# TalShor/SciLMM

Measured on AMD Instinct MI355X. Metric: REML factorize+solve nnz(L)/s (simulated pedigree, fp64), higher is better.
Workload: dtype f64

## Files before the change

scilmm_amd/_lib.py:

```python
import ctypes as C
import os

import numpy as np

_HERE = os.path.dirname(os.path.abspath(__file__))
LIB_PATH = os.environ.get("SCILMM_HIP_LIB", os.path.join(_HERE, "csrc", "libscilmm_hip.so"))

OK, ERR_ARG, ERR_NOT_PD, ERR_DEVICE, ERR_STATE = 0, -1, -2, -3, -4
DOSAGE_U16, DOSAGE_F32 = 0, 1


class ScilmmError(RuntimeError):
    pass


class NotPositiveDefiniteError(ScilmmError):

    def __init__(self, column):
        super().__init__("matrix is not positive definite (failing permuted column %d)" % column)
        self.column = column


class Options(C.Structure):
    _fields_ = [("ordering", C.c_int32), ("relax_small", C.c_int32), ("relax_w1", C.c_int32),
# ... 192 lines not shown

def check(status, sym=None, bad_col=None):
    if status == OK:
        return
    if status == ERR_NOT_PD:
        raise NotPositiveDefiniteError(-1 if bad_col is None else int(bad_col))
    msg = {ERR_ARG: "invalid argument", ERR_DEVICE: "HIP device error", ERR_STATE: "invalid call order"}.get(
        status, "error %d" % status)
    if sym:
        detail = lib().scilmm_symbolic_error(sym)
        if detail:
            msg += ": " + detail.decode()
    raise ScilmmError(msg)


def ptr(a):
    return a.ctypes.data_as(C.c_void_p)


_GET_DTYPES = {"sn_rowptr": np.int64, "sn_loff": np.int64, "asm_dst": np.int64, "diag_dst": np.int64,
               "upd_ptr": np.int64, "tile_base": np.int64, "combo_ptr": np.int64, "level_tile_ptr": np.int64,
               "level_pair_ptr": np.int64, "child_ptr": np.int64, "tail_blk_ptr": np.int64, "pat_colptr": np.int64, "inv_off": np.int64,
               "pat_rowptr": np.int64, "pat_rowslot": np.int64, "pull_seg_ptr": np.int64, "pull_level_ptr": np.int64,
               "pull_fold_ptr": np.int64}


def symbolic_get(sym, name):
    n = C.c_int64(0)
    check(lib().scilmm_symbolic_get(sym, name.encode(), None, C.byref(n)), sym)
    out = np.empty(n.value, dtype=np.int64 if name.startswith("val_") else _GET_DTYPES.get(name, np.int32))
    check(lib().scilmm_symbolic_get(sym, name.encode(), ptr(out), C.byref(n)), sym)
    return out


COMM_FN = C.CFUNCTYPE(C.c_int, C.c_void_p, C.c_int32, C.c_int32, C.c_int64, C.c_int64, C.c_int32)

ORDER_METHODS = {"amd": 0, "nesdis": 1, "nesdis_always": 2}


def order(A, method="amd"):
    indptr = np.ascontiguousarray(A.indptr, dtype=np.int64)
    indices = np.ascontiguousarray(A.indices, dtype=np.int32)
    perm = np.empty(A.shape[0], dtype=np.int32)
    check(lib().scilmm_order(A.shape[0], ptr(indptr), ptr(indices), ORDER_METHODS[method], ptr(perm)))
    return perm


# ... 69 lines not shown
```

scilmm_amd/csrc/capi_symbolic.cpp:

```cpp
#include <cstdlib>
#include <cstring>
#include <exception>
#include <memory>
#include <string>
#include <vector>

#include "../../include/scilmm_hip.h"
#include "handles.h"
#include "host_threads.h"

using scilmm::Symbolic;

static bool env_deterministic() {
  const char* e = getenv("SCILMM_DETERMINISTIC");
  return e && e[0] == '1';
}

extern "C" {

int scilmm_symbolic_create(int32_t n, int32_t K, const int64_t* const* indptr, const int32_t* const* indices,
                           const int32_t* perm_in, const scilmm_options* opts, int32_t ngpus, scilmm_symbolic** out) {
  scilmm::use_host_threads();
  if (!out || n < 0 || K <= 0 || !indptr || !indices || ngpus < 1) return SCILMM_ERR_ARG;
  scilmm::SymbolicOptions o;
  if (opts) {
    o.ordering = opts->ordering;
    if (opts->relax_small >= 0) o.relax_small = opts->relax_small;
    if (opts->relax_w1 >= 0) o.relax_w1 = opts->relax_w1;
    if (opts->relax_w2 >= 0) o.relax_w2 = opts->relax_w2;
    if (opts->relax_z1 >= 0) o.relax_z1 = opts->relax_z1;
    if (opts->relax_z2 >= 0) o.relax_z2 = opts->relax_z2;
    if (opts->relax_z3 >= 0) o.relax_z3 = opts->relax_z3;
// ... 110 lines not shown
  try {
    if (!h->S->combos_built && !std::strncmp(what, "combo_", 6)) scilmm::build_tile_combos(h->S, nullptr);
    if (!std::strncmp(what, "pull_", 5)) scilmm::build_pull_schedule(h->S);
    if (!std::strcmp(what, "pat_rowptr") || !std::strcmp(what, "pat_rowslot") || !std::strcmp(what, "pat_rowcol"))
      if (!scilmm::build_row_index(h->S)) return SCILMM_ERR_STATE;
  } catch (const std::exception& e) {
    const_cast<scilmm_symbolic*>(h)->err = e.what();
    return SCILMM_ERR_STATE;
  }
  const Symbolic& S = *h->S;
  if (!std::strcmp(what, "dense_first")) {
    if (out) *(int32_t*)out = S.dense_first;
    *count = 1;
    return SCILMM_OK;
  }
  if (!std::strncmp(what, "val_slot:", 9) || !std::strncmp(what, "val_src:", 8)) {
    const bool slot = what[4] == 's' && what[5] == 'l';
    const int k = std::atoi(what + (slot ? 9 : 8));
    if (k < 0 || k >= S.K) return SCILMM_ERR_ARG;
    const std::vector<int64_t>& v = slot ? S.val_slot[k] : S.val_src[k];
    if (out) std::memcpy(out, v.data(), v.size() * sizeof(int64_t));
    *count = (int64_t)v.size();
    return SCILMM_OK;
  }
  GET("perm", perm)
  GET("iperm", iperm)
  GET("parent", parent)
  GET("colcount", colcount)
  GET("sn_start", sn_start)
  GET("sn_parent", sn_parent)
  GET("sn_rowptr", sn_rowptr)
  GET("sn_rows", sn_rows)
  GET("sn_loff", sn_loff)
  GET("sn_level", sn_level)
  GET("level_ptr", level_ptr)
  GET("level_fronts", level_fronts)
  GET("asm_dst", asm_dst)
  GET("diag_dst", diag_dst)
  GET("upd_ptr", upd_ptr)
  GET("upd_src", upd_src)
  GET("upd_p0", upd_p0)
  GET("upd_p1", upd_p1)
  GET("tile_base", tile_base)
  GET("tile_front", tile_front)
  GET("combo_ptr", combo_ptr)
  GET("combo_pair", combo_pair)
// ... 85 lines not shown
```

scilmm_amd/csrc/dev.h:

```cpp
#pragma once
#include <hip/hip_runtime.h>

#include <algorithm>
#include <cstdlib>
#include <optional>
#include <string>
#include <type_traits>
#include <vector>

#include "../../include/scilmm_hip.h"
#include "plan_types.h"
#include "handles.h"

namespace scilmm {

struct Tuning {
  int reserve_cus = 0;
  int side_streams = 2;
  bool no_mfma = false;
  bool trsm_lite = true;
  std::optional<bool> dense;
  std::optional<bool> outside;
  bool outside_merge = true;
  std::optional<int> outside_chunks;
  bool outside_prio = false;
  std::optional<double> cell_limit;
  bool no_lookahead = false;
  int look_depth = 2;
  bool host_cells = false;
  bool no_splitk = false;
  int64_t target_items = 1024;
  int64_t min_item = 24;
  int64_t max_item = 96;
  std::optional<int64_t> dense_items;
  int64_t dense_fill = 256;
  std::optional<bool> dense_taper;
  std::optional<int> dist_group;
  bool dist_nosplit = false;
  int chain_cap = 2048;
  int chain_wide = 12;
  bool no_chain = false;
  int64_t push_slice = 512;
  bool shadow = true;
  bool dense_feed = true;
  int chain_wide_t = 160;
  int chain_full_t = 768;
  bool chain_pipe = true;
  int chain_stagger = 0;
// ... 6 lines not shown
  const char* gate = getenv("SCILMM_TUNING");
  const char* e = getenv("SCILMM_DENSE_FEED");
  return !(gate && gate[0] == '1' && e && e[0] == '0');
}

inline Tuning read_tuning() {
  Tuning t;
  t.dense_feed = read_dense_feed();
  const char* gate = getenv("SCILMM_TUNING");
  if (!(gate && gate[0] == '1')) return t;
  auto env = [](const char* name) { return getenv(name); };
  auto is1 = [&](const char* name) { const char* e = env(name); return e && e[0] == '1'; };
  auto not0 = [&](const char* name) { const char* e = env(name); return !(e && e[0] == '0'); };
  const char* e;
  if ((e = env("SCILMM_RESERVE_CUS"))) t.reserve_cus = atoi(e);
  if ((e = env("SCILMM_SIDE_STREAMS"))) t.side_streams = atoi(e);
  t.no_mfma = is1("SCILMM_NO_MFMA");
  t.trsm_lite = not0("SCILMM_TRSM_LITE");
  if ((e = env("SCILMM_DENSE"))) t.dense = e[0] != '0';
  if ((e = env("SCILMM_OUTSIDE"))) t.outside = e[0] != '0';
  t.outside_merge = not0("SCILMM_OUTSIDE_MERGE");
  if ((e = env("SCILMM_OUTSIDE_CHUNKS"))) t.outside_chunks = atoi(e);
  t.outside_prio = is1("SCILMM_OUTSIDE_PRIO");
  if ((e = env("SCILMM_CELL_LIMIT"))) t.cell_limit = atof(e);
  t.no_lookahead = is1("SCILMM_NO_LOOKAHEAD");
  if ((e = env("SCILMM_LOOK_DEPTH"))) t.look_depth = std::max(1, atoi(e));
  t.host_cells = is1("SCILMM_HOST_CELLS");
  t.no_splitk = is1("SCILMM_NO_SPLITK");
  if ((e = env("SCILMM_TARGET_ITEMS"))) t.target_items = atoll(e);
  if ((e = env("SCILMM_MIN_ITEM"))) t.min_item = atoll(e);
  if ((e = env("SCILMM_MAX_ITEM"))) t.max_item = atoll(e);
  if ((e = env("SCILMM_DENSE_ITEMS"))) t.dense_items = atoll(e);
  if ((e = env("SCILMM_DENSE_FILL"))) t.dense_fill = atoll(e);
  if ((e = env("SCILMM_DENSE_TAPER"))) t.dense_taper = e[0] == '1';
  if ((e = env("SCILMM_DIST_GROUP"))) t.dist_group = atoi(e);
  t.dist_nosplit = is1("SCILMM_DIST_NOSPLIT");
  if ((e = env("SCILMM_CHAIN_CAP"))) t.chain_cap = atoi(e);
  if ((e = env("SCILMM_CHAIN_WIDE"))) t.chain_wide = atoi(e);
  t.no_chain = is1("SCILMM_NO_CHAIN");
  if ((e = env("SCILMM_PUSH_SLICE"))) t.push_slice = atoll(e);
  t.shadow = not0("SCILMM_SHADOW");
  if ((e = env("SCILMM_CHAIN_WIDE_T"))) t.chain_wide_t = atoi(e);
  if ((e = env("SCILMM_CHAIN_FULL_T"))) t.chain_full_t = atoi(e);
  t.chain_pipe = not0("SCILMM_CHAIN_PIPE");
  if ((e = env("SCILMM_CHAIN_STAGGER"))) t.chain_stagger = std::max(0, atoi(e));
  t.sinv_generic = is1("SCILMM_SINV_GENERIC");
// ... 128 lines not shown
  int32_t* d_col_front = nullptr;
  int64_t* d_yoff = nullptr;
  double* d_ybuf = nullptr;
  int32_t* d_sinv_pre_tiles = nullptr;
  std::vector<int64_t> sinv_pre_ptr;
  std::vector<int32_t> sinv_tail_front;
  int32_t* d_sinv_tail_fronts = nullptr;
  SinvWork* d_sinv_work = nullptr;
  std::vector<int64_t> sinv_work_ptr;
  std::vector<int32_t> sinv_tail_nseg;
  double* d_sinv_tail_partial = nullptr;
  SinvSeg* d_sinv_cc_segs = nullptr;
  std::vector<int64_t> sinv_cc_seg_ptr;
  SinvFold* d_sinv_cc_folds = nullptr;
  std::vector<int64_t> sinv_cc_fold_ptr;
  double* d_sinv_cc_partial = nullptr;
  bool work_external = false;
  bool outside_on = false;
  int32_t tail_level = 0;
  std::vector<uint8_t> outside_desc;
  OutsideWork* d_owork = nullptr;
  int32_t* d_grp_next = nullptr;
  int32_t* d_grp_t0 = nullptr;
  int64_t n_owork = 0;
  int32_t* d_tail_front = nullptr;
  uint8_t* d_keep_front = nullptr;
  hipStream_t outside_st = nullptr;
  std::vector<int64_t> ochunk_ptr;
  std::vector<hipEvent_t> out_evs;
  std::vector<int32_t> out_wait_chunk;
  bool dense_on = false;
  int front_bits = 64;
  double* d_zeros = nullptr;
  DenseWork* d_dwork_e = nullptr;
  DenseWork* d_dwork_l = nullptr;
  std::vector<int64_t> dwork_e_ptr, dwork_l_ptr;
  std::vector<int64_t> dwork_l_mid;
  int64_t n_late_split = 0;
  int look_depth = 2;
  int rhs_pending = -1;
  int32_t chain_T = 0, chain_l0 = 0;
  int32_t* d_chain = nullptr;
  int32_t* d_colmap = nullptr;
  int32_t* d_cf_ptr = nullptr;
  ChainPair* d_cf = nullptr;
  int32_t* d_cb_ptr = nullptr;
// ... 178 lines not shown
```

scilmm_amd/csrc/kernels.hip.h:

```cpp
#pragma once
#include <hip/hip_runtime.h>
#ifndef SCILMM_UPD_WAVES
#define SCILMM_UPD_WAVES 2
#endif
#include <stdint.h>
#include <type_traits>

#include "plan_types.h"

namespace scilmm {

typedef double d4 __attribute__((ext_vector_type(4)));

constexpr int NJB = NB / 16;
constexpr int KCS = 16;
constexpr int LDA = TM + 16;
constexpr int LDB = NB + 16;
constexpr int LDP = 34;

__device__ __forceinline__ d4 mfma_f64(double a, double b, d4 c) {
  return __builtin_amdgcn_mfma_f64_16x16x4f64(a, b, c, 0, 0, 0);
}

__global__ void k_assemble(int64_t nnz, const int64_t* __restrict__ dst, ValPtrs vp, double* __restrict__ L) {
// ... 842 lines not shown
#endif
  double* P = L + S.sn_loff[j];
#pragma unroll
  for (int jb = 0; jb < NJH; ++jb)
#pragma unroll
    for (int ib = 0; ib < 2; ++ib)
#pragma unroll
      for (int r = 0; r < 4; ++r) {
        const int i = ia + ib, jc = 64 * ch + 16 * jb + 4 * lk + r;
#ifdef SCILMM_DENSE_H_NOFOLD
        const double v = (double)c32[jb][ib][r];
#else
        const double v = acc[jb][ib][r];
#endif
        if (slot < 0) {
          if (i < nrow && jc < wj) P[(int64_t)jc * mj + R0 + i] -= v;
        } else {
          scratch[(int64_t)slot * (TM * NB) + jc * TM + i] = v;
        }
      }
}

template <bool MFMA, int SCATTER = 0>
__global__ __launch_bounds__(256) void k_outside(DevSym S, int32_t dense_first, const OutsideWork* __restrict__ work,
                                                 const int32_t* __restrict__ tail_front,
                                                 const uint8_t* __restrict__ keep_front,
                                                 const int32_t* __restrict__ grp_next,
                                                 const int32_t* __restrict__ grp_t0,
                                                 double* __restrict__ L) {
  __shared__ __attribute__((aligned(16))) double As[KCS * LDA];
  __shared__ __attribute__((aligned(16))) double Bs[KCS * LDB];
  __shared__ int32_t lab_i[TM], lab_j[NB];
  const int tid = threadIdx.x, lane = tid & 63, wv = tid >> 6;
  const OutsideWork wk = work[blockIdx.x];
  int32_t ni, nj;
  {
    const int32_t d = wk.d;
    const int32_t md = (int32_t)(S.sn_rowptr[d + 1] - S.sn_rowptr[d]);
    const int32_t* rd = S.sn_rows + S.sn_rowptr[d];
    const int32_t ri0 = wk.t0 + TM * wk.bi, rj0 = wk.t0 + NB * wk.bj;
    ni = min(TM, md - ri0);
    nj = min(NB, md - rj0);
    if (tid < TM) lab_i[tid] = tid < ni ? rd[ri0 + tid] : -1;
    else if (tid < TM + NB) lab_j[tid - TM] = (tid - TM) < nj ? rd[rj0 + tid - TM] : -1;
  }
  d4 acc[NJB][2];
#pragma unroll
  for (int a = 0; a < NJB; ++a) { acc[a][0] = (d4){0.0, 0.0, 0.0, 0.0}; acc[a][1] = (d4){0.0, 0.0, 0.0, 0.0}; }
  const int x = tid & 127, kk = tid >> 7;
  bool first_chunk = true;
  for (int32_t d = wk.d, t0 = wk.t0; d >= 0;) {
    const int32_t wd = S.sn_start[d + 1] - S.sn_start[d];
    const int32_t md = (int32_t)(S.sn_rowptr[d + 1] - S.sn_rowptr[d]);
    const double* Pd = L + S.sn_loff[d];
    const int32_t ri0 = t0 + TM * wk.bi, rj0 = t0 + NB * wk.bj;
    const double* pa = Pd + ri0 + min(x, ni - 1);
    const double* pb = Pd + rj0 + min(x, nj - 1);
    for (int32_t k0 = 0; k0 < wd; k0 += KCS) {
      const int kc = min(KCS, wd - k0);
      const int kc4 = (kc + 3) & ~3;
      double va[KCS / 2], vb[KCS / 2];
#pragma unroll
      for (int i = 0; i < KCS / 2; ++i) {
        const int64_t kq = k0 + min(kk + 2 * i, kc - 1);
        va[i] = pa[kq * md];
        vb[i] = pb[kq * md];
      }
      if (!first_chunk) __syncthreads();
      first_chunk = false;
#pragma unroll
      for (int i = 0; i < KCS / 2; ++i) {
        const int k = kk + 2 * i;
        if (k < kc4) {
          As[k * LDA + x] = (x < ni && k < kc) ? va[i] : 0.0;
          Bs[k * LDB + x] = (x < nj && k < kc) ? vb[i] : 0.0;
        }
      }
      __syncthreads();
      if (32 * wv < ni) tile_mma<MFMA>(As, Bs, kc4, NJB, lane, wv, acc);
    }
    d = grp_next[d];
    if (d >= 0) t0 = grp_t0[d];
  }
  const int li = lane & 15, lr = lane >> 4;
  const int32_t c0_tail = S.sn_start[dense_first];
#pragma unroll
  for (int jb = 0; jb < NJB; ++jb)
#pragma unroll
    for (int r = 0; r < 4; ++r) {
      const int jloc = 16 * jb + lr + 4 * r;
      const int32_t cj = lab_j[jloc];
      if (cj < 0) continue;
      const int32_t f = tail_front[cj - c0_tail];
      if (!keep_front[f]) continue;
      const int32_t c0f = S.sn_start[f];
      double* col = L + S.sn_loff[f] + (int64_t)(cj - c0f) * (S.n - c0f) - c0f;
#pragma unroll
      for (int ib = 0; ib < 2; ++ib) {
        const int iloc = 32 * wv + 16 * ib + li;
        const int32_t ci = lab_i[iloc];
        if (SCATTER == 0) {
          if (ci >= cj) unsafeAtomicAdd(col + ci, -acc[jb][ib][r]);
        } else if (SCATTER == 1) {
          if (ci >= cj && acc[jb][ib][r] == 123.456) col[ci] = 0.0;
        } else {
          if (ci >= cj) col[ci] = -acc[jb][ib][r];
        }
      }
    }
}


__device__ __forceinline__ double cell_dot(const double* __restrict__ L, int64_t st, int64_t sq, int64_t md, int wd) {
  const double* pt = L + st;
  const double* pq = L + sq;
  double acc = 0.0;
  int k = 0;
  for (; k + 8 <= wd; k += 8) {
    double a[8], b[8];
#pragma unroll
    for (int u = 0; u < 8; ++u) {
      a[u] = pt[(int64_t)(k + u) * md];
      b[u] = pq[(int64_t)(k + u) * md];
    }
    double s0 = 0.0, s1 = 0.0;
#pragma unroll
    for (int u = 0; u < 8; u += 2) {
      s0 += a[u] * b[u];
      s1 += a[u + 1] * b[u + 1];
    }
    acc += s0 + s1;
  }
// ... 2356 lines not shown
```

scilmm_amd/csrc/launch.hip.h:

```cpp
#pragma once

namespace {

int set_attrs(scilmm_symbolic* sym, Dev* D) {
  if (D->attrs_set) return SCILMM_OK;
  const int big = 150 * 1024;
  HIPCHK(hipFuncSetAttribute((const void*)k_potrf, hipFuncAttributeMaxDynamicSharedMemorySize, big));
  HIPCHK(hipFuncSetAttribute((const void*)k_fwd<true, 0, true>, hipFuncAttributeMaxDynamicSharedMemorySize, big));
  HIPCHK(hipFuncSetAttribute((const void*)k_fwd<true, 0, false>, hipFuncAttributeMaxDynamicSharedMemorySize, big));
  HIPCHK(hipFuncSetAttribute((const void*)k_fwd<true, 1, true>, hipFuncAttributeMaxDynamicSharedMemorySize, big));
  HIPCHK(hipFuncSetAttribute((const void*)k_fwd<false, 0, true>, hipFuncAttributeMaxDynamicSharedMemorySize, big));
  HIPCHK(hipFuncSetAttribute((const void*)k_fwd<false, 0, false>, hipFuncAttributeMaxDynamicSharedMemorySize, big));
  HIPCHK(hipFuncSetAttribute((const void*)k_fwd<false, 1, true>, hipFuncAttributeMaxDynamicSharedMemorySize, big));
  HIPCHK(hipFuncSetAttribute((const void*)k_dense32, hipFuncAttributeMaxDynamicSharedMemorySize, big));
  HIPCHK(hipFuncSetAttribute((const void*)k_dense_h, hipFuncAttributeMaxDynamicSharedMemorySize, big));
  HIPCHK(hipFuncSetAttribute((const void*)k_dense_b<2>, hipFuncAttributeMaxDynamicSharedMemorySize, big));
  HIPCHK(hipFuncSetAttribute((const void*)k_dense_b<0>, hipFuncAttributeMaxDynamicSharedMemorySize, big));
  HIPCHK(hipFuncSetAttribute((const void*)k_update2<true>, hipFuncAttributeMaxDynamicSharedMemorySize, big));
  HIPCHK(hipFuncSetAttribute((const void*)k_update2<false>, hipFuncAttributeMaxDynamicSharedMemorySize, big));
  D->attrs_set = true;
  return SCILMM_OK;
}

inline int64_t max_groups(unsigned threads) { return (int64_t)(((uint64_t)1 << 32) / threads) - 1; }
// ... 62 lines not shown
                       (const int32_t*)CS.wd, fac->L);
    launches++;
    return SCILMM_OK;
  }

  void trsm(hipStream_t stream, const int32_t* tiles, int64_t cnt, const double* slabs) {
    const bool lite = D->use_mfma && D->trsm_lite;
    const auto k = lite ? k_trsm_lite : D->use_mfma ? k_trsm<true> : k_trsm<false>;
    const int64_t per = lite ? max_groups(256) / 4 : max_groups(256);
    for (int64_t o = 0; o < cnt; o += per) {
      const int64_t c = std::min(cnt - o, per);
      hipLaunchKernelGGL(k, dim3((unsigned)(lite ? 4 * c : c)), dim3(256), 0, stream, D->v, tiles + o, fac->L, fac->invD, D->d_tile_pslot,
                         D->d_tile_pnseg, slabs);
      launches++;
    }
  }

  void outside(hipStream_t stream, const OutsideWork* work, int64_t cnt) {
    auto k = D->use_mfma ? k_outside<true> : k_outside<false>;
#ifdef SCILMM_DIAG
    if (D->ablate == 6) k = k_outside<true, 1>;
    if (D->ablate == 7) k = k_outside<true, 2>;
#endif
    for (int64_t o = 0; o < cnt; o += max_groups(256)) {
      const unsigned c = (unsigned)std::min<int64_t>(max_groups(256), cnt - o);
      hipLaunchKernelGGL(k, dim3(c), dim3(256), 0, stream, D->v, fac->sym->S->dense_first, work + o, D->d_tail_front, D->d_keep_front,
                         D->d_grp_next, D->d_grp_t0, fac->L);
      launches++;
      D->n_float_atomic++;
    }
  }
};

struct SweepLaunch {
  Dev* const D;
  const scilmm_factor* const fac;
  const hipStream_t st;
  int rp = 0;
  unsigned gy = 1;

  void diag_solve(bool trans, const int32_t* fronts, int64_t cnt, const double* in, double* out) const {
    if (cnt <= 0) return;
    const auto k = D->use_mfma ? (trans ? k_diag_solve<true, true> : k_diag_solve<true, false>)
                               : (trans ? k_diag_solve<false, true> : k_diag_solve<false, false>);
    hipLaunchKernelGGL(k, dim3((unsigned)cnt, gy), dim3(256), 0, st, D->v, fronts, fac->invD, in, out, rp);
  }

  void fwd(int mode, bool atomic, const int32_t* tiles, int64_t cnt, const double* in, double* out) const {
    if (cnt <= 0) return;
    const size_t sm_fwd = sizeof(double) * (size_t)(NB * LDW + KCS * LDA);
// ... 87 lines not shown
```

scilmm_amd/csrc/plan.hip:

```cpp
#include <hip/hip_runtime.h>

#include <algorithm>
#include <atomic>
#include <chrono>
#include <functional>
#include <thread>
#include <cmath>
#include <cstdio>
#include <cstdlib>
#include <cstring>
#include <string>
#include <vector>

#include "dev.h"
#include "cellplan.hip.h"
#include "host_threads.h"

namespace scilmm {

void dev_free(void* p) {
  Dev* D = (Dev*)p;
  if (!D) return;
  for (void* a : D->allocs) (void)hipFree(a);
  for (double* v : D->vals)
// ... 390 lines not shown
  const Symbolic& S = *sym->S;
  const int32_t tail_w = tail_width(S);
  {
    D->dense_on = S.dense_first < S.nsuper && D->use_mfma && D->tune.dense.value_or(tail_w >= 8192);
    if (distributed_tail(D, S)) D->dense_on = true;
    if (D->dense_on && !D->d_zeros) {
      HIPCHK(hipMalloc((void**)&D->d_zeros, 2048));
      HIPCHK(hipMemset(D->d_zeros, 0, 2048));
    }
  }
  {
    D->outside_desc.assign((size_t)std::max(S.nsuper, 1), 0);
    D->outside_on = S.dense_first < S.nsuper && !D->det && !sym->S->combos_built && D->tune.outside.value_or(tail_w >= 8192);
  }
  return SCILMM_OK;
}

int plan_outside(scilmm_symbolic* sym, Dev* D, PlanBuild& pb) {
  const Symbolic& S = *sym->S;
  int st = SCILMM_OK;
  D->tail_level = S.sn_level[S.dense_first];
  const int32_t c0_tail = S.sn_start[S.dense_first];
  std::vector<OutsideWork> ow;
  std::vector<int32_t> grp_next((size_t)std::max(S.nsuper, 1), -1), grp_t0((size_t)std::max(S.nsuper, 1), 0);
  std::vector<int32_t> grp_width((size_t)std::max(S.nsuper, 1), 0);
  {
    const bool merge = D->tune.outside_merge;
    std::vector<std::pair<uint64_t, int32_t>> keyed;
    for (int32_t d = 0; d < S.dense_first; ++d) {
      if (S.sn_level[d] >= D->tail_level) continue;
      const int32_t* rd = S.sn_rows.data() + S.sn_rowptr[d];
      const int32_t md = (int32_t)(S.sn_rowptr[d + 1] - S.sn_rowptr[d]);
      const int32_t t0 = (int32_t)(std::lower_bound(rd, rd + md, c0_tail) - rd);
      if (t0 >= md) continue;
      D->outside_desc[d] = 1;
      grp_t0[(size_t)d] = t0;
      uint64_t h = 1469598103934665603ull ^ (uint64_t)(md - t0);
      for (int32_t t = t0; t < md; ++t) h = (h ^ (uint64_t)(uint32_t)rd[t]) * 1099511628211ull;
      keyed.push_back({merge ? h : (uint64_t)d, d});
    }
    std::stable_sort(keyed.begin(), keyed.end(), [](const std::pair<uint64_t, int32_t>& a, const std::pair<uint64_t, int32_t>& b) { return a.first < b.first; });
    auto same_rows = [&](int32_t a, int32_t b) -> bool {
      const int64_t na = S.sn_rowptr[a + 1] - S.sn_rowptr[a] - grp_t0[(size_t)a], nb = S.sn_rowptr[b + 1] - S.sn_rowptr[b] - grp_t0[(size_t)b];
      return na == nb && std::memcmp(S.sn_rows.data() + S.sn_rowptr[a] + grp_t0[(size_t)a], S.sn_rows.data() + S.sn_rowptr[b] + grp_t0[(size_t)b],
                                     sizeof(int32_t) * (size_t)na) == 0;
    };
    std::vector<int32_t> leaders;
    for (size_t i = 0; i < keyed.size();) {
      size_t j = i;
      while (j < keyed.size() && keyed[j].first == keyed[i].first) ++j;
      std::vector<uint8_t> used(j - i, 0);
      for (size_t a = i; a < j; ++a) {
        if (used[a - i]) continue;
        const int32_t lead = keyed[a].second;
        leaders.push_back(lead);
        int32_t last = lead;
        grp_width[(size_t)lead] = S.sn_start[lead + 1] - S.sn_start[lead];
        for (size_t b = a + 1; b < j; ++b) {
          if (used[b - i] || !merge || !same_rows(lead, keyed[b].second)) continue;
          used[b - i] = 1;
          grp_next[(size_t)last] = keyed[b].second;
          last = keyed[b].second;
          grp_width[(size_t)lead] += S.sn_start[last + 1] - S.sn_start[last];
        }
      }
      i = j;
    }
    std::sort(leaders.begin(), leaders.end());
    const bool own_only = distributed_tail(D, S);
    int64_t pairs_all = 0;
    for (int32_t d : leaders) {
      const int32_t md = (int32_t)(S.sn_rowptr[d + 1] - S.sn_rowptr[d]), t0 = grp_t0[(size_t)d];
      const int32_t* rd = S.sn_rows.data() + S.sn_rowptr[d];
      const int32_t nb = (md - t0 + TM - 1) / TM;
      std::vector<uint8_t> col_mine((size_t)nb, 1);
      if (own_only)
        for (int32_t bj = 0; bj < nb; ++bj) {
          const int32_t r_lo = rd[t0 + NB * bj], r_hi = rd[std::min(md, t0 + NB * (bj + 1)) - 1];
          int32_t f_lo = (int32_t)(std::upper_bound(S.sn_start.begin() + S.dense_first, S.sn_start.begin() + S.nsuper + 1, r_lo) - S.sn_start.begin()) - 1;
          int32_t f_hi = (int32_t)(std::upper_bound(S.sn_start.begin() + S.dense_first, S.sn_start.begin() + S.nsuper + 1, r_hi) - S.sn_start.begin()) - 1;
          uint8_t mine = 0;
          for (int32_t f = f_lo; f <= f_hi && !mine; ++f) mine = D->keep_front[(size_t)f];
          col_mine[(size_t)bj] = mine;
        }
      for (int32_t bi = 0; bi < nb; ++bi)
        for (int32_t bj = 0; bj <= bi; ++bj) {
          ++pairs_all;
          if (col_mine[(size_t)bj]) ow.push_back(OutsideWork{d, t0, bi, bj});
        }
    }
    if (pb.verbose)
      fprintf(stderr, "[scilmm plan] k_outside: %zu descendants in %zu groups of identical tail rows; %lld of %lld block pairs reach a panel of this rank\n",
              keyed.size(), leaders.size(), (long long)ow.size(), (long long)pairs_all);
  }
  D->n_owork = (int64_t)ow.size();
  if (D->n_owork == 0 || D->tail_level == 0) {
    D->outside_on = false;
    std::fill(D->outside_desc.begin(), D->outside_desc.end(), 0);
  } else {
    std::vector<int32_t> tf((size_t)(S.n - c0_tail));
    for (int32_t f = S.dense_first; f < S.nsuper; ++f)
      for (int32_t c = S.sn_start[f]; c < S.sn_start[f + 1]; ++c) tf[(size_t)(c - c0_tail)] = f;
    auto first_front = [&](const OutsideWork& w) -> int32_t {
      return tf[(size_t)(S.sn_rows[S.sn_rowptr[w.d] + w.t0 + NB * w.bj] - c0_tail)];
    };
    const int32_t want_chunks = std::max(1, D->tune.outside_chunks.value_or((int32_t)std::min<int64_t>(32, std::max<int64_t>(4, (int64_t)ow.size() / 16384))));
    std::vector<int32_t> ffront(ow.size());
    for (size_t i = 0; i < ow.size(); ++i) ffront[i] = first_front(ow[i]);
    std::vector<size_t> ord(ow.size());
    for (size_t i = 0; i < ord.size(); ++i) ord[i] = i;
    std::stable_sort(ord.begin(), ord.end(), [&](size_t a, size_t b) { return ffront[a] < ffront[b]; });
    D->ochunk_ptr.assign(1, 0);
    std::vector<int32_t> chunk_lo;
    {
      const size_t N = ord.size();
      size_t panels = N ? 1 : 0;
      for (size_t k = 1; k < N; ++k) panels += ffront[ord[k]] != ffront[ord[k - 1]];
      const size_t per = (size_t)want_chunks >= panels ? 1 : std::max<size_t>(1, (N + want_chunks - 1) / want_chunks);
      size_t i = 0;
      while (i < N) {
        chunk_lo.push_back(ffront[ord[i]]);
        size_t e = std::min(N, i + per);
        while (e < N && ffront[ord[e]] == ffront[ord[e - 1]]) ++e;
        D->ochunk_ptr.push_back((int64_t)e);
        i = e;
      }
    }
    const int32_t nch = (int32_t)chunk_lo.size();
    {
      std::vector<OutsideWork> sorted(ow.size());
      for (int32_t g = 0; g < nch; ++g) {
        std::stable_sort(ord.begin() + D->ochunk_ptr[g], ord.begin() + D->ochunk_ptr[g + 1], [&](size_t a, size_t b) {
          return grp_width[(size_t)ow[a].d] > grp_width[(size_t)ow[b].d];
        });
      }
      for (size_t i = 0; i < ord.size(); ++i) sorted[i] = ow[ord[i]];
      ow.swap(sorted);
    }
    D->out_wait_chunk.assign((size_t)std::max(S.nlevels, 1), -1);
    for (int32_t f = S.dense_first; f < S.nsuper; ++f) {
      const int32_t g = (int32_t)(std::upper_bound(chunk_lo.begin(), chunk_lo.end(), f) - chunk_lo.begin()) - 1;
      int32_t& w = D->out_wait_chunk[(size_t)S.sn_level[f]];
      w = std::max(w, g);
    }
    for (int32_t l = D->tail_level + 1; l < S.nlevels; ++l)
      D->out_wait_chunk[(size_t)l] = std::max(D->out_wait_chunk[(size_t)l], D->out_wait_chunk[(size_t)l - 1]);
    D->out_evs.assign((size_t)nch, nullptr);
    for (auto& e : D->out_evs) HIPCHK(hipEventCreateWithFlags(&e, hipEventDisableTiming));
    if ((st = upload(sym, D, ow, &D->d_owork)) != SCILMM_OK) return st;
    {
      if ((st = upload(sym, D, grp_next, &D->d_grp_next)) != SCILMM_OK) return st;
      if ((st = upload(sym, D, grp_t0, &D->d_grp_t0)) != SCILMM_OK) return st;
    }
    if ((st = upload(sym, D, tf, &D->d_tail_front)) != SCILMM_OK) return st;
    if ((st = upload(sym, D, D->keep_front, &D->d_keep_front)) != SCILMM_OK) return st;
    {
      HIPCHK(hipStreamCreateWithPriority(&D->outside_st, hipStreamNonBlocking, D->tune.outside_prio ? D->prio_hi : D->prio_lo));
    }
    if (pb.verbose) {
      fprintf(stderr, "[scilmm plan] k_outside: %lld block-pair items of prelude fronts below level %d (tail starts at column %d), %d chunks by first panel:",
              (long long)D->n_owork, D->tail_level, c0_tail, nch);
      for (int32_t g = 0; g < nch; ++g) fprintf(stderr, " [%d..: %lld]", chunk_lo[g] - S.dense_first, (long long)(D->ochunk_ptr[g + 1] - D->ochunk_ptr[g]));
      fprintf(stderr, "\n");
      fprintf(stderr, "[scilmm plan] k_outside: on a stream of %s priority\n", D->tune.outside_prio ? "the chain's" : "the look-ahead streams'");
    }
  }
  return SCILMM_OK;
}

int upload_symbolic(scilmm_symbolic* sym, Dev* D) {
  const Symbolic& S = *sym->S;
  const std::vector<int64_t>& LOFF = D->loff;
  D->v.n = S.n;
  D->v.nsuper = S.nsuper;
  int st;
// ... 1266 lines not shown
```

Before: 1.450 billion.

## Nest outside-update groups whose tail rows are subsets of an ancestor group

Groups of prelude descendants whose tail row set is a subset of a parent group's rows (above a size ratio) are chained into the root group's accumulation. Per-member index maps gather the right rows, so one tile scatter covers several groups and fewer atomic adds reach L. Work items of nested leaders are marked dead, and the kernel becomes grid-stride with an optional capped grid. The cost is more planning work on the host, extra map lookups inside the kernel, and zero-padded rows that lower MFMA efficiency.

```diff
diff --git a/scilmm_amd/_lib.py b/scilmm_amd/_lib.py
--- a/scilmm_amd/_lib.py
+++ b/scilmm_amd/_lib.py
@@ -238,7 +238,7 @@
                "upd_ptr": np.int64, "tile_base": np.int64, "combo_ptr": np.int64, "level_tile_ptr": np.int64,
                "level_pair_ptr": np.int64, "child_ptr": np.int64, "tail_blk_ptr": np.int64, "pat_colptr": np.int64, "inv_off": np.int64,
                "pat_rowptr": np.int64, "pat_rowslot": np.int64, "pull_seg_ptr": np.int64, "pull_level_ptr": np.int64,
-               "pull_fold_ptr": np.int64}
+               "pull_fold_ptr": np.int64, "outside_map_off": np.int64, "outside_counts": np.int64}
 
 
 def symbolic_get(sym, name):
diff --git a/scilmm_amd/csrc/capi_symbolic.cpp b/scilmm_amd/csrc/capi_symbolic.cpp
--- a/scilmm_amd/csrc/capi_symbolic.cpp
+++ b/scilmm_amd/csrc/capi_symbolic.cpp
@@ -8,6 +8,7 @@
 #include "../../include/scilmm_hip.h"
 #include "handles.h"
 #include "host_threads.h"
+#include "outside_groups.h"
 
 using scilmm::Symbolic;
 
@@ -164,6 +165,27 @@
     if (out) std::memcpy(out, v.data(), v.size() * sizeof(int64_t));
     *count = (int64_t)v.size();
     return SCILMM_OK;
+  }
+  if (!std::strncmp(what, "outside_", 8)) {
+    const scilmm::OutsideSwitches sw = scilmm::read_outside_switches();
+    const scilmm::OutsideGroups G =
+        scilmm::outside_groups(S.nsuper, S.dense_first, S.sn_start.data(), S.sn_rowptr.data(), S.sn_rows.data(), S.sn_level.data(),
+                               S.sn_parent.data(), sw.merge, sw.nest);
+    const std::vector<int64_t> counts = {G.n_desc, (int64_t)G.leaders.size(), G.nested_members, G.pairs_leaders, G.pairs_scatter, G.skipped};
+    auto give = [&](const auto& v) {
+      if (out && !v.empty()) std::memcpy(out, v.data(), v.size() * sizeof(v[0]));
+      *count = (int64_t)v.size();
+      return SCILMM_OK;
+    };
+    const char* w = what + 8;
+    if (!std::strcmp(w, "root")) return give(G.root);
+    if (!std::strcmp(w, "next")) return give(G.next);
+    if (!std::strcmp(w, "t0")) return give(G.t0);
+    if (!std::strcmp(w, "map_off")) return give(G.map_off);
+    if (!std::strcmp(w, "maps")) return give(G.maps);
+    if (!std::strcmp(w, "leaders")) return give(G.leaders);
+    if (!std::strcmp(w, "counts")) return give(counts);
+    return SCILMM_ERR_ARG;
   }
   GET("perm", perm)
   GET("iperm", iperm)
diff --git a/scilmm_amd/csrc/dev.h b/scilmm_amd/csrc/dev.h
--- a/scilmm_amd/csrc/dev.h
+++ b/scilmm_amd/csrc/dev.h
@@ -11,6 +11,7 @@
 #include "../../include/scilmm_hip.h"
 #include "plan_types.h"
 #include "handles.h"
+#include "outside_groups.h"
 
 namespace scilmm {
 
@@ -24,6 +25,8 @@
   bool outside_merge = true;
   std::optional<int> outside_chunks;
   bool outside_prio = false;
+  double outside_nest = OUTSIDE_NEST_DEFAULT;
+  int outside_wgs = OUTSIDE_WGS_DEFAULT;
   std::optional<double> cell_limit;
   bool no_lookahead = false;
   int look_depth = 2;
@@ -76,6 +79,11 @@
   t.outside_merge = not0("SCILMM_OUTSIDE_MERGE");
   if ((e = env("SCILMM_OUTSIDE_CHUNKS"))) t.outside_chunks = atoi(e);
   t.outside_prio = is1("SCILMM_OUTSIDE_PRIO");
+  {
+    const OutsideSwitches os = read_outside_switches();
+    t.outside_nest = os.nest;
+    t.outside_wgs = os.wgs;
+  }
   if ((e = env("SCILMM_CELL_LIMIT"))) t.cell_limit = atof(e);
   t.no_lookahead = is1("SCILMM_NO_LOOKAHEAD");
   if ((e = env("SCILMM_LOOK_DEPTH"))) t.look_depth = std::max(1, atoi(e));
@@ -250,6 +258,8 @@
   OutsideWork* d_owork = nullptr;
   int32_t* d_grp_next = nullptr;
   int32_t* d_grp_t0 = nullptr;
+  int64_t* d_grp_map_off = nullptr;
+  int32_t* d_grp_maps = nullptr;
   int64_t n_owork = 0;
   int32_t* d_tail_front = nullptr;
   uint8_t* d_keep_front = nullptr;
diff --git a/scilmm_amd/csrc/kernels.hip.h b/scilmm_amd/csrc/kernels.hip.h
--- a/scilmm_amd/csrc/kernels.hip.h
+++ b/scilmm_amd/csrc/kernels.hip.h
@@ -888,92 +888,114 @@
 }
 
 template <bool MFMA, int SCATTER = 0>
-__global__ __launch_bounds__(256) void k_outside(DevSym S, int32_t dense_first, const OutsideWork* __restrict__ work,
+__global__ __launch_bounds__(256) void k_outside(DevSym S, int32_t dense_first, const OutsideWork* __restrict__ work, int64_t cnt,
                                                  const int32_t* __restrict__ tail_front,
                                                  const uint8_t* __restrict__ keep_front,
                                                  const int32_t* __restrict__ grp_next,
                                                  const int32_t* __restrict__ grp_t0,
+                                                 const int64_t* __restrict__ grp_map_off,
+                                                 const int32_t* __restrict__ grp_maps,
                                                  double* __restrict__ L) {
   __shared__ __attribute__((aligned(16))) double As[KCS * LDA];
   __shared__ __attribute__((aligned(16))) double Bs[KCS * LDB];
   __shared__ int32_t lab_i[TM], lab_j[NB];
   const int tid = threadIdx.x, lane = tid & 63, wv = tid >> 6;
-  const OutsideWork wk = work[blockIdx.x];
-  int32_t ni, nj;
-  {
-    const int32_t d = wk.d;
-    const int32_t md = (int32_t)(S.sn_rowptr[d + 1] - S.sn_rowptr[d]);
-    const int32_t* rd = S.sn_rows + S.sn_rowptr[d];
-    const int32_t ri0 = wk.t0 + TM * wk.bi, rj0 = wk.t0 + NB * wk.bj;
-    ni = min(TM, md - ri0);
-    nj = min(NB, md - rj0);
-    if (tid < TM) lab_i[tid] = tid < ni ? rd[ri0 + tid] : -1;
-    else if (tid < TM + NB) lab_j[tid - TM] = (tid - TM) < nj ? rd[rj0 + tid - TM] : -1;
-  }
-  d4 acc[NJB][2];
-#pragma unroll
-  for (int a = 0; a < NJB; ++a) { acc[a][0] = (d4){0.0, 0.0, 0.0, 0.0}; acc[a][1] = (d4){0.0, 0.0, 0.0, 0.0}; }
   const int x = tid & 127, kk = tid >> 7;
-  bool first_chunk = true;
-  for (int32_t d = wk.d, t0 = wk.t0; d >= 0;) {
-    const int32_t wd = S.sn_start[d + 1] - S.sn_start[d];
-    const int32_t md = (int32_t)(S.sn_rowptr[d + 1] - S.sn_rowptr[d]);
-    const double* Pd = L + S.sn_loff[d];
-    const int32_t ri0 = t0 + TM * wk.bi, rj0 = t0 + NB * wk.bj;
-    const double* pa = Pd + ri0 + min(x, ni - 1);
-    const double* pb = Pd + rj0 + min(x, nj - 1);
-    for (int32_t k0 = 0; k0 < wd; k0 += KCS) {
-      const int kc = min(KCS, wd - k0);
-      const int kc4 = (kc + 3) & ~3;
-      double va[KCS / 2], vb[KCS / 2];
-#pragma unroll
-      for (int i = 0; i < KCS / 2; ++i) {
-        const int64_t kq = k0 + min(kk + 2 * i, kc - 1);
-        va[i] = pa[kq * md];
-        vb[i] = pb[kq * md];
-      }
-      if (!first_chunk) __syncthreads();
-      first_chunk = false;
-#pragma unroll
-      for (int i = 0; i < KCS / 2; ++i) {
-        const int k = kk + 2 * i;
-        if (k < kc4) {
-          As[k * LDA + x] = (x < ni && k < kc) ? va[i] : 0.0;
-          Bs[k * LDB + x] = (x < nj && k < kc) ? vb[i] : 0.0;
-        }
-      }
-      __syncthreads();
-      if (32 * wv < ni) tile_mma<MFMA>(As, Bs, kc4, NJB, lane, wv, acc);
-    }
-    d = grp_next[d];
-    if (d >= 0) t0 = grp_t0[d];
-  }
-  const int li = lane & 15, lr = lane >> 4;
   const int32_t c0_tail = S.sn_start[dense_first];
-#pragma unroll
-  for (int jb = 0; jb < NJB; ++jb)
-#pragma unroll
-    for (int r = 0; r < 4; ++r) {
-      const int jloc = 16 * jb + lr + 4 * r;
-      const int32_t cj = lab_j[jloc];
-      if (cj < 0) continue;
-      const int32_t f = tail_front[cj - c0_tail];
-      if (!keep_front[f]) continue;
-      const int32_t c0f = S.sn_start[f];
-      double* col = L + S.sn_loff[f] + (int64_t)(cj - c0f) * (S.n - c0f) - c0f;
-#pragma unroll
-      for (int ib = 0; ib < 2; ++ib) {
-        const int iloc = 32 * wv + 16 * ib + li;
-        const int32_t ci = lab_i[iloc];
-        if (SCATTER == 0) {
-          if (ci >= cj) unsafeAtomicAdd(col + ci, -acc[jb][ib][r]);
-        } else if (SCATTER == 1) {
-          if (ci >= cj && acc[jb][ib][r] == 123.456) col[ci] = 0.0;
-        } else {
-          if (ci >= cj) col[ci] = -acc[jb][ib][r];
-        }
-      }
-    }
+  bool touched = false;
+  for (int64_t item = blockIdx.x; item < cnt; item += gridDim.x) {
+    const OutsideWork wk = work[item];
+    if (wk.t0 < 0) continue;
+    if (touched) __syncthreads();
+    touched = true;
+    int32_t ni, nj, tr;
+    {
+      const int32_t d = wk.d;
+      const int32_t md = (int32_t)(S.sn_rowptr[d + 1] - S.sn_rowptr[d]);
+      const int32_t* rd = S.sn_rows + S.sn_rowptr[d];
+      const int32_t ri0 = wk.t0 + TM * wk.bi, rj0 = wk.t0 + NB * wk.bj;
+      tr = md - wk.t0;
+      ni = min(TM, md - ri0);
+      nj = min(NB, md - rj0);
+      if (tid < TM) lab_i[tid] = tid < ni ? rd[ri0 + tid] : -1;
+      else if (tid < TM + NB) lab_j[tid - TM] = (tid - TM) < nj ? rd[rj0 + tid - TM] : -1;
+    }
+    d4 acc[NJB][2];
+#pragma unroll
+    for (int a = 0; a < NJB; ++a) { acc[a][0] = (d4){0.0, 0.0, 0.0, 0.0}; acc[a][1] = (d4){0.0, 0.0, 0.0, 0.0}; }
+    bool first_chunk = true;
+    for (int32_t d = wk.d, t0 = wk.t0; d >= 0;) {
+      const int32_t wd = S.sn_start[d + 1] - S.sn_start[d];
+      const int32_t md = (int32_t)(S.sn_rowptr[d + 1] - S.sn_rowptr[d]);
+      const double* Pd = L + S.sn_loff[d];
+      int32_t ra = t0 + TM * wk.bi + min(x, ni - 1), rb = t0 + NB * wk.bj + min(x, nj - 1);
+      bool oka = x < ni, okb = x < nj, skip = false;
+      const int64_t mo = grp_map_off[d];
+      if (mo >= 0) {
+        const int32_t* mp = grp_maps + mo;
+        skip = !(mp[tr + wk.bi] && mp[tr + wk.bj]);
+        if (!skip) {
+          const int32_t qa = oka ? mp[TM * wk.bi + x] : -1, qb = okb ? mp[NB * wk.bj + x] : -1;
+          oka = qa >= 0;
+          okb = qb >= 0;
+          ra = t0 + max(qa, 0);
+          rb = t0 + max(qb, 0);
+        }
+      }
+      const double* pa = Pd + ra;
+      const double* pb = Pd + rb;
+      for (int32_t k0 = 0; k0 < wd && !skip; k0 += KCS) {
+        const int kc = min(KCS, wd - k0);
+        const int kc4 = (kc + 3) & ~3;
+        double va[KCS / 2], vb[KCS / 2];
+#pragma unroll
+        for (int i = 0; i < KCS / 2; ++i) {
+          const int64_t kq = k0 + min(kk + 2 * i, kc - 1);
+          va[i] = pa[kq * md];
+          vb[i] = pb[kq * md];
+        }
+        if (!first_chunk) __syncthreads();
+        first_chunk = false;
+#pragma unroll
+        for (int i = 0; i < KCS / 2; ++i) {
+          const int k = kk + 2 * i;
+          if (k < kc4) {
+            As[k * LDA + x] = (oka && k < kc) ? va[i] : 0.0;
+            Bs[k * LDB + x] = (okb && k < kc) ? vb[i] : 0.0;
+          }
+        }
+        __syncthreads();
+        if (32 * wv < ni) tile_mma<MFMA>(As, Bs, kc4, NJB, lane, wv, acc);
+      }
+      d = grp_next[d];
+      if (d >= 0) t0 = grp_t0[d];
+    }
+    const int li = lane & 15, lr = lane >> 4;
+#pragma unroll
+    for (int jb = 0; jb < NJB; ++jb)
+#pragma unroll
+      for (int r = 0; r < 4; ++r) {
+        const int jloc = 16 * jb + lr + 4 * r;
+        const int32_t cj = lab_j[jloc];
+        if (cj < 0) continue;
+        const int32_t f = tail_front[cj - c0_tail];
+        if (!keep_front[f]) continue;
+        const int32_t c0f = S.sn_start[f];
+        double* col = L + S.sn_loff[f] + (int64_t)(cj - c0f) * (S.n - c0f) - c0f;
+#pragma unroll
+        for (int ib = 0; ib < 2; ++ib) {
+          const int iloc = 32 * wv + 16 * ib + li;
+          const int32_t ci = lab_i[iloc];
+          if (SCATTER == 0) {
+            if (ci >= cj) unsafeAtomicAdd(col + ci, -acc[jb][ib][r]);
+          } else if (SCATTER == 1) {
+            if (ci >= cj && acc[jb][ib][r] == 123.456) col[ci] = 0.0;
+          } else {
+            if (ci >= cj) col[ci] = -acc[jb][ib][r];
+          }
+        }
+      }
+  }
 }
 
 
diff --git a/scilmm_amd/csrc/launch.hip.h b/scilmm_amd/csrc/launch.hip.h
--- a/scilmm_amd/csrc/launch.hip.h
+++ b/scilmm_amd/csrc/launch.hip.h
@@ -108,10 +108,12 @@
     if (D->ablate == 6) k = k_outside<true, 1>;
     if (D->ablate == 7) k = k_outside<true, 2>;
 #endif
+    const int64_t wgs = D->tune.outside_wgs;
     for (int64_t o = 0; o < cnt; o += max_groups(256)) {
-      const unsigned c = (unsigned)std::min<int64_t>(max_groups(256), cnt - o);
-      hipLaunchKernelGGL(k, dim3(c), dim3(256), 0, stream, D->v, fac->sym->S->dense_first, work + o, D->d_tail_front, D->d_keep_front,
-                         D->d_grp_next, D->d_grp_t0, fac->L);
+      const int64_t c = std::min<int64_t>(max_groups(256), cnt - o);
+      const unsigned grid = (unsigned)(wgs > 0 ? std::min(wgs, c) : c);
+      hipLaunchKernelGGL(k, dim3(grid), dim3(256), 0, stream, D->v, fac->sym->S->dense_first, work + o, c, D->d_tail_front, D->d_keep_front,
+                         D->d_grp_next, D->d_grp_t0, D->d_grp_map_off, D->d_grp_maps, fac->L);
       launches++;
       D->n_float_atomic++;
     }
diff --git a/scilmm_amd/csrc/outside_groups.h b/scilmm_amd/csrc/outside_groups.h
--- /dev/null
+++ b/scilmm_amd/csrc/outside_groups.h
@@ -0,0 +1,169 @@
+#pragma once
+#include <algorithm>
+#include <cstdint>
+#include <cstdlib>
+#include <cstring>
+#include <utility>
+#include <vector>
+
+namespace scilmm {
+
+constexpr double OUTSIDE_NEST_DEFAULT = 0.5;
+constexpr int OUTSIDE_WGS_DEFAULT = 0;
+struct OutsideSwitches {
+  bool merge = true;
+  double nest = OUTSIDE_NEST_DEFAULT;
+  int wgs = OUTSIDE_WGS_DEFAULT;
+};
+inline OutsideSwitches read_outside_switches() {
+  OutsideSwitches s;
+  const char* gate = getenv("SCILMM_TUNING");
+  if (!(gate && gate[0] == '1')) return s;
+  const char* e;
+  if ((e = getenv("SCILMM_OUTSIDE_MERGE"))) s.merge = e[0] != '0';
+  if ((e = getenv("SCILMM_OUTSIDE_NEST"))) s.nest = std::min(1.0, std::max(0.0, atof(e)));
+  if ((e = getenv("SCILMM_OUTSIDE_WGS"))) s.wgs = std::max(0, atoi(e));
+  return s;
+}
+
+struct OutsideGroups {
+  std::vector<uint8_t> desc;
+  std::vector<int32_t> t0;
+  std::vector<int32_t> next;
+  std::vector<int32_t> root;
+  std::vector<int64_t> map_off;
+  std::vector<int32_t> width;
+  std::vector<int32_t> leaders;
+  std::vector<uint8_t> nested_leader;
+  std::vector<int32_t> maps;
+  int64_t n_desc = 0;
+  int64_t nested_members = 0;
+  int64_t pairs_leaders = 0;
+  int64_t pairs_scatter = 0;
+  int64_t skipped = 0;
+};
+
+inline int32_t outside_blocks(int32_t t, int32_t tm) { return (t + tm - 1) / tm; }
+inline int64_t outside_lower_pairs(int32_t nb) { return (int64_t)nb * (nb + 1) / 2; }
+
+inline OutsideGroups outside_groups(int32_t nsuper, int32_t dense_first, const int32_t* sn_start, const int64_t* sn_rowptr,
+                                    const int32_t* sn_rows, const int32_t* sn_level, const int32_t* sn_parent, bool merge, double phi,
+                                    int32_t tm = 128) {
+  OutsideGroups G;
+  const size_t ns = (size_t)std::max(nsuper, 1);
+  G.desc.assign(ns, 0);
+  G.t0.assign(ns, 0);
+  G.next.assign(ns, -1);
+  G.root.assign(ns, -1);
+  G.map_off.assign(ns, -1);
+  G.width.assign(ns, 0);
+  if (dense_first >= nsuper) return G;
+  const int32_t tail_level = sn_level[dense_first], c0_tail = sn_start[dense_first];
+  auto tail_rows = [&](int32_t d) { return sn_rows + sn_rowptr[d] + G.t0[(size_t)d]; };
+  auto tail_count = [&](int32_t d) { return (int32_t)(sn_rowptr[d + 1] - sn_rowptr[d]) - G.t0[(size_t)d]; };
+  std::vector<std::pair<uint64_t, int32_t>> keyed;
+  for (int32_t d = 0; d < dense_first; ++d) {
+    if (sn_level[d] >= tail_level) continue;
+    const int32_t* rd = sn_rows + sn_rowptr[d];
+    const int32_t md = (int32_t)(sn_rowptr[d + 1] - sn_rowptr[d]);
+    const int32_t t0 = (int32_t)(std::lower_bound(rd, rd + md, c0_tail) - rd);
+    if (t0 >= md) continue;
+    G.desc[(size_t)d] = 1;
+    G.t0[(size_t)d] = t0;
+    uint64_t h = 1469598103934665603ull ^ (uint64_t)(md - t0);
+    for (int32_t t = t0; t < md; ++t) h = (h ^ (uint64_t)(uint32_t)rd[t]) * 1099511628211ull;
+    keyed.push_back({merge ? h : (uint64_t)d, d});
+  }
+  G.n_desc = (int64_t)keyed.size();
+  std::stable_sort(keyed.begin(), keyed.end(),
+                   [](const std::pair<uint64_t, int32_t>& a, const std::pair<uint64_t, int32_t>& b) { return a.first < b.first; });
+  auto same_rows = [&](int32_t a, int32_t b) -> bool {
+    const int32_t na = tail_count(a), nb = tail_count(b);
+    return na == nb && std::memcmp(tail_rows(a), tail_rows(b), sizeof(int32_t) * (size_t)na) == 0;
+  };
+  std::vector<int32_t> leader_of(ns, -1), last_of(ns, -1);
+  for (size_t i = 0; i < keyed.size();) {
+    size_t j = i;
+    while (j < keyed.size() && keyed[j].first == keyed[i].first) ++j;
+    std::vector<uint8_t> used(j - i, 0);
+    for (size_t a = i; a < j; ++a) {
+      if (used[a - i]) continue;
+      const int32_t lead = keyed[a].second;
+      G.leaders.push_back(lead);
+      int32_t last = lead;
+      leader_of[(size_t)lead] = lead;
+      G.width[(size_t)lead] = sn_start[lead + 1] - sn_start[lead];
+      for (size_t b = a + 1; b < j; ++b) {
+        if (used[b - i] || !merge || !same_rows(lead, keyed[b].second)) continue;
+        used[b - i] = 1;
+        G.next[(size_t)last] = keyed[b].second;
+        last = keyed[b].second;
+        leader_of[(size_t)last] = lead;
+        G.width[(size_t)lead] += sn_start[last + 1] - sn_start[last];
+      }
+      last_of[(size_t)lead] = last;
+    }
+    i = j;
+  }
+  std::sort(G.leaders.begin(), G.leaders.end());
+  for (int32_t g : G.leaders) {
+    G.root[(size_t)g] = g;
+    G.pairs_leaders += outside_lower_pairs(outside_blocks(tail_count(g), tm));
+  }
+  std::vector<int32_t> chain_last(last_of);
+  if (merge && phi > 0.0) {
+    std::vector<int32_t> by_top(G.leaders);
+    std::sort(by_top.begin(), by_top.end(), [&](int32_t a, int32_t b) { return last_of[(size_t)a] > last_of[(size_t)b]; });
+    for (int32_t g : by_top) {
+      const int32_t p = sn_parent[last_of[(size_t)g]];
+      if (p < 0 || p >= dense_first || !G.desc[(size_t)p]) continue;
+      const int32_t r = G.root[(size_t)leader_of[(size_t)p]];
+      const int32_t tg = tail_count(g), tr = tail_count(r);
+      if (r == g || (double)tg < phi * (double)tr) continue;
+      if (!std::includes(tail_rows(r), tail_rows(r) + tr, tail_rows(g), tail_rows(g) + tg)) continue;
+      G.root[(size_t)g] = r;
+    }
+  }
+  G.nested_leader.assign(G.leaders.size(), 0);
+  for (size_t li = 0; li < G.leaders.size(); ++li) {
+    const int32_t g = G.leaders[li], r = G.root[(size_t)g];
+    if (r == g) continue;
+    G.nested_leader[li] = 1;
+    const int32_t tg = tail_count(g), tr = tail_count(r), nb = outside_blocks(tr, tm);
+    const int64_t off = (int64_t)G.maps.size();
+    G.maps.resize((size_t)(off + tr + nb), 0);
+    int32_t* mp = G.maps.data() + off;
+    const int32_t *Tr = tail_rows(r), *Tg = tail_rows(g);
+    int32_t q = 0;
+    for (int32_t i = 0; i < tr; ++i) {
+      if (q < tg && Tg[q] == Tr[i]) {
+        mp[i] = q++;
+        mp[tr + i / tm] = 1;
+      } else {
+        mp[i] = -1;
+      }
+    }
+    G.next[(size_t)chain_last[(size_t)r]] = g;
+    chain_last[(size_t)r] = last_of[(size_t)g];
+    G.width[(size_t)r] += G.width[(size_t)g];
+    int64_t skip_items = 0;
+    for (int32_t bi = 0; bi < nb; ++bi)
+      for (int32_t bj = 0; bj <= bi; ++bj) skip_items += !(mp[tr + bi] && mp[tr + bj]);
+    for (int32_t m = g; m >= 0 && leader_of[(size_t)m] == g; m = G.next[(size_t)m]) {
+      G.root[(size_t)m] = r;
+      G.map_off[(size_t)m] = off;
+      ++G.nested_members;
+      G.skipped += skip_items;
+      if (m == last_of[(size_t)g]) break;
+    }
+  }
+  for (size_t li = 0; li < G.leaders.size(); ++li) {
+    const int32_t g = G.leaders[li];
+    if (G.nested_leader[li]) continue;
+    for (int32_t m = g; m >= 0 && G.map_off[(size_t)m] < 0; m = G.next[(size_t)m]) G.root[(size_t)m] = g;
+    G.pairs_scatter += outside_lower_pairs(outside_blocks(tail_count(g), tm));
+  }
+  return G;
+}
+
+}
diff --git a/scilmm_amd/csrc/plan.hip b/scilmm_amd/csrc/plan.hip
--- a/scilmm_amd/csrc/plan.hip
+++ b/scilmm_amd/csrc/plan.hip
@@ -436,51 +436,12 @@
   D->tail_level = S.sn_level[S.dense_first];
   const int32_t c0_tail = S.sn_start[S.dense_first];
   std::vector<OutsideWork> ow;
-  std::vector<int32_t> grp_next((size_t)std::max(S.nsuper, 1), -1), grp_t0((size_t)std::max(S.nsuper, 1), 0);
-  std::vector<int32_t> grp_width((size_t)std::max(S.nsuper, 1), 0);
+  const OutsideGroups og = outside_groups(S.nsuper, S.dense_first, S.sn_start.data(), S.sn_rowptr.data(), S.sn_rows.data(), S.sn_level.data(),
+                                          S.sn_parent.data(), D->tune.outside_merge, D->tune.outside_nest, TM);
+  const std::vector<int32_t>&grp_next = og.next, &grp_t0 = og.t0, &grp_width = og.width;
   {
-    const bool merge = D->tune.outside_merge;
-    std::vector<std::pair<uint64_t, int32_t>> keyed;
-    for (int32_t d = 0; d < S.dense_first; ++d) {
-      if (S.sn_level[d] >= D->tail_level) continue;
-      const int32_t* rd = S.sn_rows.data() + S.sn_rowptr[d];
-      const int32_t md = (int32_t)(S.sn_rowptr[d + 1] - S.sn_rowptr[d]);
-      const int32_t t0 = (int32_t)(std::lower_bound(rd, rd + md, c0_tail) - rd);
-      if (t0 >= md) continue;
-      D->outside_desc[d] = 1;
-      grp_t0[(size_t)d] = t0;
-      uint64_t h = 1469598103934665603ull ^ (uint64_t)(md - t0);
-      for (int32_t t = t0; t < md; ++t) h = (h ^ (uint64_t)(uint32_t)rd[t]) * 1099511628211ull;
-      keyed.push_back({merge ? h : (uint64_t)d, d});
-    }
-    std::stable_sort(keyed.begin(), keyed.end(), [](const std::pair<uint64_t, int32_t>& a, const std::pair<uint64_t, int32_t>& b) { return a.first < b.first; });
-    auto same_rows = [&](int32_t a, int32_t b) -> bool {
-      const int64_t na = S.sn_rowptr[a + 1] - S.sn_rowptr[a] - grp_t0[(size_t)a], nb = S.sn_rowptr[b + 1] - S.sn_rowptr[b] - grp_t0[(size_t)b];
-      return na == nb && std::memcmp(S.sn_rows.data() + S.sn_rowptr[a] + grp_t0[(size_t)a], S.sn_rows.data() + S.sn_rowptr[b] + grp_t0[(size_t)b],
-                                     sizeof(int32_t) * (size_t)na) == 0;
-    };
-    std::vector<int32_t> leaders;
-    for (size_t i = 0; i < keyed.size();) {
-      size_t j = i;
-      while (j < keyed.size() && keyed[j].first == keyed[i].first) ++j;
-      std::vector<uint8_t> used(j - i, 0);
-      for (size_t a = i; a < j; ++a) {
-        if (used[a - i]) continue;
-        const int32_t lead = keyed[a].second;
-        leaders.push_back(lead);
-        int32_t last = lead;
-        grp_width[(size_t)lead] = S.sn_start[lead + 1] - S.sn_start[lead];
-        for (size_t b = a + 1; b < j; ++b) {
-          if (used[b - i] || !merge || !same_rows(lead, keyed[b].second)) continue;
-          used[b - i] = 1;
-          grp_next[(size_t)last] = keyed[b].second;
-          last = keyed[b].second;
-          grp_width[(size_t)lead] += S.sn_start[last + 1] - S.sn_start[last];
-        }
-      }
-      i = j;
-    }
-    std::sort(leaders.begin(), leaders.end());
+    D->outside_desc = og.desc;
+    const std::vector<int32_t>& leaders = og.leaders;
     const bool own_only = distributed_tail(D, S);
     int64_t pairs_all = 0;
     for (int32_t d : leaders) {
@@ -505,7 +466,10 @@
     }
     if (pb.verbose)
       fprintf(stderr, "[scilmm plan] k_outside: %zu descendants in %zu groups of identical tail rows; %lld of %lld block pairs reach a panel of this rank\n",
-              keyed.size(), leaders.size(), (long long)ow.size(), (long long)pairs_all);
+              (size_t)og.n_desc, leaders.size(), (long long)ow.size(), (long long)pairs_all);
+    if (pb.verbose)
+      fprintf(stderr, "[scilmm plan] k_outside: %lld nested members (tail rows a subset of their root's, phi %.2f), %lld scattering block pairs, %lld skipped (member, block pair)\n",
+              (long long)og.nested_members, D->tune.outside_nest, (long long)og.pairs_scatter, (long long)og.skipped);
   }
   D->n_owork = (int64_t)ow.size();
   if (D->n_owork == 0 || D->tail_level == 0) {
@@ -550,6 +514,8 @@
       }
       for (size_t i = 0; i < ord.size(); ++i) sorted[i] = ow[ord[i]];
       ow.swap(sorted);
+      for (OutsideWork& w : ow)
+        if (og.root[(size_t)w.d] != w.d) w.t0 = -1;
     }
     D->out_wait_chunk.assign((size_t)std::max(S.nlevels, 1), -1);
     for (int32_t f = S.dense_first; f < S.nsuper; ++f) {
@@ -565,6 +531,8 @@
     {
       if ((st = upload(sym, D, grp_next, &D->d_grp_next)) != SCILMM_OK) return st;
       if ((st = upload(sym, D, grp_t0, &D->d_grp_t0)) != SCILMM_OK) return st;
+      if ((st = upload(sym, D, og.map_off, &D->d_grp_map_off)) != SCILMM_OK) return st;
+      if ((st = upload(sym, D, og.maps, &D->d_grp_maps)) != SCILMM_OK) return st;
     }
     if ((st = upload(sym, D, tf, &D->d_tail_front)) != SCILMM_OK) return st;
     if ((st = upload(sym, D, D->keep_front, &D->d_keep_front)) != SCILMM_OK) return st;
```

Result: no change. 1.464 billion (median of 6 runs) (+1.0%).
